# sipposip/pr-disagg-radar-gan

Hardware: AMD Instinct MI355X
Metric: cWGAN-GP train samples/sec, 24x16x16 tiles, bs=256 (higher is better)
Workload: dtype f32; 1 GPU; ndomain=16, 24h, bs=256 fp32, 1 critic step + 1 gen step (BASELINE configs[1]); batch_per_gpu=256, global_batch=256, n_critic=1, parallelism=dp1, world=1, rccl_ranks_seen=1, weights=random init (RandomNormal 0.02 / glorot_uniform), dropout 0.25 active

## Files before the change

### pr_disagg_radar_gan_amd/csrc/rdgan_api.hip

```cpp
#include <hip/hip_runtime.h>
#include <stdio.h>
#include <string.h>
#include <math.h>
#include <string>
#include <vector>
#include <algorithm>
#include <unordered_set>

#include "../../include/rdgan.h"
#include "rdgan_plan.h"
#include "rdgan_hostplan.h"
#include "rdgan_rng.h"
#include "rdgan_gemm.hip.h"
#include "rdgan_gemm_ws.hip.h"
#include "rdgan_gemm_ws16.hip.h"
#include "rdgan_gemm_f16.hip.h"
#include "rdgan_upconv16.hip.h"
#include "rdgan_upconv16b.hip.h"
#include "rdgan_upconv16t.hip.h"
#include "rdgan_elem.hip.h"
#include "rdgan_data.hip.h"
#include "rdgan_edge.hip.h"
#include "rdgan_d2slab16.hip.h"
#include "rdgan_d2fwd16.hip.h"
// ... 63 lines not shown
  int wgrad_boxes = 1;
  int border_boxes = 1;
  int d2_gate_bits = 1;
  int d2_slab = 1;
  int a16 = 0;
  int g9_direct = 1;
  int fast_fwd = -1;
  int fast_bwd = -1;
  float *GWC[4], *GWD[4], *dWc;
  int collapse = 1;
  int tapgather = 1;
  int ws_ksplit = 1;
  int wave_spec = 1;
  int resident = 1;
  int edge_kernels = 1;
  int sample_offset = 0;
  float* g9b_tmp;
  float* gp_part;
  float* dw6_part;
  int side_on = 1;
  int split3 = 0;
  int dense_slices = 0;
  uint64_t gver_in = 0, cver_in = 0;
  const float* gcache_ptr = nullptr; uint64_t gcache_ver = 0; int gcache_cfg = -1;
  const float* ccache_ptr = nullptr; uint64_t ccache_ver = 0; int ccache_cfg = -1;
  long form_builds[2] = {0, 0};
  int keep_gates = 0;
  void* gate_keep[5] = {nullptr, nullptr, nullptr, nullptr, nullptr};
  int gate_keep_B = 0;
  hipStream_t side = nullptr;
  hipEvent_t ev_fork = nullptr, ev_join = nullptr, ev_cw = nullptr, ev_g[4] = {nullptr, nullptr, nullptr, nullptr};
  int* d_flag;
  int fwd_ahead = -1;
  hipStream_t ahead = nullptr;
  hipEvent_t ev_ahead_fork = nullptr, ev_ahead_done = nullptr;
  float* kpartial_ahead = nullptr;
  int* flag_ahead = nullptr;
  bool ahead_pending = false;
  const float *ahead_gp = nullptr, *ahead_z = nullptr, *ahead_cond = nullptr;
  int ahead_B = 0;
  uint64_t ahead_gver = 0;
  std::unordered_set<const void*> lds_attr_done;
  int prof_launches = 0;
  std::vector<RdLaunchRec> launch_recs;
  size_t launch_used = 0;
  char cur_kernel[48] = {0};
  double flops_acc = 0;
  unsigned prof_mask = 0;
  std::vector<hipEvent_t> ev_start[RDGAN_NUM_TAGS], ev_stop[RDGAN_NUM_TAGS];
  size_t ev_used[RDGAN_NUM_TAGS] = {0};
};

#define RD_CHECK(h, call)                                                        \
  do {                                                                           \
    hipError_t e_ = (call);                                                      \
    if (e_ != hipSuccess) {                                                      \
      char b_[512];                                                              \
      snprintf(b_, sizeof b_, "%s:%d %s -> %s", __FILE__, __LINE__, #call, hipGetErrorString(e_)); \
      if (h) (h)->err = b_;                                                      \
      return (int)e_;                                                            \
    }                                                                            \
  } while (0)
#define RD_TRY(expr)            \
  do {                          \
    int r_ = (expr);            \
    if (r_ != 0) return r_;     \
// ... 418 lines not shown
  const bool ws = h && h->wave_spec && !partial && !shift && !dy16 && (h->wave_spec == 2 || wrows * hp.nphases >= 1024 || T.box);
  const bool direct = !ws && !T.box && !dy16 && !partial && np == 1 && nsplit == 1 && h != nullptr && hp.ph[0].w_off == 0;
  if (direct) { T.direct = 1; T.ldw = hp.N; partial_buf = dW; }
  if (dy16) {
    if (shift || BR != 64 || BN != 64) return bad_arg(h, "wgrad: bf16 output gradient only with the 64x64 tile");
    if (partial) RD_TRY((launch_wgrad_cfg<64, 64, true, false, true>(h, dp, np, B, src, dy, partial_buf, T, nsplit, st)));
    else RD_TRY((launch_wgrad_cfg<64, 64, false, false, true>(h, dp, np, B, src, dy, partial_buf, T, nsplit, st)));
  }
  else if (ws && BR == 256) RD_TRY((launch_wgrad_ws_cfg<256, 64>(h, dp, np, B, src, dy, partial_buf, T, nsplit, st)));
  else if (ws && BR == 128 && BN == 128) RD_TRY((launch_wgrad_ws_cfg<128, 128>(h, dp, np, B, src, dy, partial_buf, T, nsplit, st)));
  else if (ws && BR == 128) RD_TRY((launch_wgrad_ws_cfg<128, 64>(h, dp, np, B, src, dy, partial_buf, T, nsplit, st)));
  else if (ws && BN == 128) RD_TRY((launch_wgrad_ws_cfg<64, 128>(h, dp, np, B, src, dy, partial_buf, T, nsplit, st)));
  else if (ws) RD_TRY((launch_wgrad_ws_cfg<64, 64>(h, dp, np, B, src, dy, partial_buf, T, nsplit, st)));
  else if (partial) RD_TRY((launch_wgrad_cfg<64, 64, true, false>(h, dp, np, B, src, dy, partial_buf, T, nsplit, st)));
  else if (BR == 256) RD_WG(256, 64);
  else if (BR == 128 && BN == 128) RD_WG(128, 128);
  else if (BR == 128) RD_WG(128, 64);
  else if (BN == 128) RD_WG(64, 128);
  else RD_WG(64, 64);
#undef RD_WG
  if (direct) { RD_CHECK(h, hipGetLastError()); return 0; }
  if (T.box) {
    const int nw = 64 - __builtin_clzll(hp.wmask | 1ull);
    const long nout = (long)nw * hp.SC * (hp.N / 4);
    hipLaunchKernelGGL(k_wgrad_reduce_box, dim3((unsigned)((nout + 255) / 256)), dim3(256), 0, st, dp, partial_ws, T, BR, B, nw, dW, hp.N);
    RD_CHECK(h, hipGetLastError());
    return 0;
  }
  long total = (long)T.RT * BR * (hp.N / 4);
  int outs = 256;
  while (outs > 16 && (total + outs - 1) / outs * np < 512 && 256 / outs < nsplit) outs >>= 1;
  hipLaunchKernelGGL(k_wgrad_reduce, dim3((unsigned)((total + outs - 1) / outs), np), dim3(256), 0, st, dp, partial_ws,
                     nsplit, T, BR, dW, hp.N, outs);
  RD_CHECK(h, hipGetLastError());
  return 0;
}

template <int BR, int BN>
static int launch_wgrad16_cfg(rdgan_handle* h, const RdPlan* dp, int nphases, int B, const void* src16, const void* dy16,
                              float* partial, const RdWgradTiling& T, int nsplit, hipStream_t st) {
  constexpr size_t lds_loop = ((BR == 256 && BN == 128) ? 3 : 2) * (size_t)(64 * BR * 2 + 64 * BN * 2);
  constexpr size_t lds_epi = (size_t)BR * BN * sizeof(float);
  constexpr size_t lds = lds_loop > lds_epi ? lds_loop : lds_epi;
  auto kern = k_wgrad_gemm_ws16<BR, BN>;
  RD_KNAME(h, "k_wgrad_gemm_ws16<%d,%d>", BR, BN);
  RD_TRY(ensure_lds(h, (const void*)kern, lds));
  dim3 grid((unsigned)(T.box ? T.nsplit : T.RT * T.NT * nsplit * nphases));
  hipLaunchKernelGGL(kern, grid, dim3(512), lds, st, dp, B, (const unsigned short*)src16, (const unsigned short*)dy16, partial, T);
  RD_CHECK(h, hipGetLastError());
  return 0;
}
static bool wgrad16_ok(const RdPlan& hp, int B) {
  int BR, BN, nsplit;
  if (hp.s_shift || hp.SC % 64 || hp.N % 64) return false;
  wgrad_tiling(hp, B, BR, BN, nsplit);
  return BR >= 128;
}
static bool wgrad16_wide(const rdgan_handle* h) { return !h || h->wgrad_wide; }
static int launch_wgrad16(rdgan_handle* h, const RdPlan& hp, const RdPlan* dp, int B, const void* src16, const void* dy16,
                          float* dW, float* partial_ws, size_t partial_cap, hipStream_t st, int tag) {
  ProfScope ps(h, tag, st);
  LaunchScope ls(h, plan_index(h, hp), RD_KIND_WGRAD, B, plan_flops(hp, B), st);
  if (h) h->flops_acc += plan_flops(hp, B);
  if (!wgrad16_ok(hp, B)) return bad_arg(h, "wgrad16: needs SC % 64 == 0, N % 64 == 0, a 128- or 256-row tile, no folded upsample");
  if (!hp.boxes)
  for (int i = 1; i < hp.nphases; ++i)
// ... 337 lines not shown
  if (!strcmp(name, "upconv_slab_t")) { h->upconv_slab_t = value ? 1 : 0; return 0; }
  if (!strcmp(name, "upconv2_slab")) { h->upconv2_slab = value ? 1 : 0; return 0; }
  if (!strcmp(name, "g9_fused")) { h->g9_fused = value ? 1 : 0; return 0; }
  if (!strcmp(name, "d1_fwd_sample")) { h->d1_fwd_sample = value ? 1 : 0; return 0; }
  if (!strcmp(name, "g9_bwd_mfma")) { h->g9_bwd_mfma = value ? 1 : 0; return 0; }
  if (!strcmp(name, "dense16")) { h->dense16 = value ? 1 : 0; return 0; }
  if (!strcmp(name, "dense_skinny")) { h->dense_skinny = value ? 1 : 0; return 0; }
  if (!strcmp(name, "wgrad_boxes")) { h->wgrad_boxes = value ? 1 : 0; return 0; }
  if (!strcmp(name, "border_boxes")) { h->border_boxes = value < 0 ? 0 : (value > 2 ? 2 : value); return 0; }
  if (!strcmp(name, "d3_wgrad_slab")) { h->d3_wgrad_slab = value ? 1 : 0; return 0; }
  if (!strcmp(name, "d2_wgrad_slab")) { h->d2_wgrad_slab = value ? 1 : 0; return 0; }
  if (!strcmp(name, "upwgrad_slab")) { h->upwgrad_slab = value ? 1 : 0; return 0; }
  if (!strcmp(name, "d1_dgrad_fused")) { h->d1_dgrad_fused = value ? 1 : 0; return 0; }
  if (!strcmp(name, "d1_wgrad16")) { h->d1_wgrad16 = value ? 1 : 0; return 0; }
  if (!strcmp(name, "wgrad_wide")) { h->wgrad_wide = value ? 1 : 0; return 0; }
  if (!strcmp(name, "conv_f16")) {
    if (value < 0 || value > 2) return bad_arg(h, "conv_f16: 0, 1 or 2 (2: regardless of the launch size)");
    h->conv_f16 = value; h->ccache_ver = 0; h->gcache_ver = 0; return 0;
  }
  if (!strcmp(name, "d2_fwd_slab")) { h->d2_fwd_slab = value ? 1 : 0; h->ccache_ver = 0; return 0; }
  if (!strcmp(name, "d2_gate_bits")) { h->d2_gate_bits = value ? 1 : 0; return 0; }
  if (!strcmp(name, "d2_slab")) { h->d2_slab = value ? 1 : 0; h->ccache_ver = 0; return 0; }
  if (!strcmp(name, "dense_wgrad_slices")) { h->dense_slices = value; return 0; }
  if (!strcmp(name, "keep_gates")) {
    h->keep_gates = value ? 1 : 0;
    h->gate_keep_B = 0;
    for (int l = 1; l <= 4 && h->keep_gates; ++l)
      if (!h->gate_keep[l]) RD_CHECK(h, hipMalloc(&h->gate_keep[l], (size_t)h->MB * h->dL[l] * h->dch[l] * sizeof(float)));
    return 0;
  }
  if (!strcmp(name, "split3")) { h->split3 = value ? 1 : 0; return 0; }
  if (!strcmp(name, "side_stream")) { h->side_on = (value && h->side) ? 1 : 0; return 0; }
  if (!strcmp(name, "gen_fwd_ahead")) { h->fwd_ahead = value < 0 ? -1 : (value ? 1 : 0); return 0; }
  if (!strcmp(name, "edge_kernels")) { h->edge_kernels = value < 0 ? 0 : (value > 2 ? 2 : value); return 0; }
  if (!strcmp(name, "sample_offset")) { if (value < 0) return bad_arg(h, "set_option: sample_offset < 0"); h->sample_offset = value; return 0; }
  if (!strcmp(name, "ws_ksplit")) { h->ws_ksplit = value < 0 ? 0 : (value > 8 ? 8 : value); return 0; }
  return bad_arg(h, "set_option: unknown option");
}

extern "C" int rdgan_set_weight_versions(rdgan_handle* h, uint64_t gen_version, uint64_t critic_version) {
  if (!h) return -2;
  h->gver_in = gen_version; h->cver_in = critic_version;
  return 0;
}
extern "C" int rdgan_form_builds(const rdgan_handle* h, long* gen_builds, long* critic_builds) {
  if (!h) return -2;
  if (gen_builds) *gen_builds = h->form_builds[0];
  if (critic_builds) *critic_builds = h->form_builds[1];
  return 0;
}

extern "C" int rdgan_profile(rdgan_handle* h, unsigned tag_mask) {
  if (!h) return -2;
  h->prof_mask = tag_mask;
  for (int t = 0; t < RDGAN_NUM_TAGS; ++t) {
    h->ev_used[t] = 0;
    if ((tag_mask >> t & 1u) && h->ev_start[t].empty()) {
      h->ev_start[t].resize(4096); h->ev_stop[t].resize(4096);
      for (size_t i = 0; i < 4096; ++i) {
        RD_CHECK(h, hipEventCreate(&h->ev_start[t][i]));
        RD_CHECK(h, hipEventCreate(&h->ev_stop[t][i]));
      }
    }
  }
  return 0;
}
// ... 1035 lines not shown
      RD_CHECK(h, hipGetLastError());
    } else if (fast) {
      ProfScope ps(h, RDGAN_TAG_ELEMENTWISE, st);
      const long HW = (long)h->gdim[l][1] * h->gdim[l][2];
      RD_TRY(launch_pn_bwd_pairs(h, l == 3 ? h->gh3 : gups[l + 1], hs[l], rs[l], dys[l], h->fgS, (long)B * h->gdim[l - 1][0] * HW,
                                 HW, h->gch[l], st, a16));
    } else {
      ProfScope ps(h, RDGAN_TAG_ELEMENTWISE, st);
      if (l == 3) RD_TRY(launch_pn_bwd(h, h->gh3, hs[3], rs[3], dys[3], npix3, 64, 0, 0, 0, 0, st, a16));
      else RD_TRY(launch_pn_bwd(h, gups[l + 1], hs[l], rs[l], dys[l], (long)B * h->gpix[l], h->gch[l], col ? 0 : 1,
                                h->gdim[l][0], h->gdim[l][1], h->gdim[l][2], st, a16));
    }
    const long cc = (long)h->gch[l - 1] * h->gch[l];
    if (fast) {
      const int* sd = h->gdim[l - 1];
      const int D = sd[0];
      const long P = (long)sd[1] * sd[2] * h->gch[l - 1];
      RdWeightMap wm;
      fastd_weight_map(wm);
      {
        ProfScope ps(h, RDGAN_TAG_ELEMENTWISE, st);
        if (!gen_block_fast(h, l, fast_fwd_on(h))) {
          const dim3 dg(ew_blocks((long)B * (D + 1) * P / 4));
          if (a16) hipLaunchKernelGGL(k_diff_d<rd_bf16_t>, dg, dim3(256), 0, st, (const rd_bf16_t*)hs[l - 1], (rd_bf16_t*)h->fE[l], B, D, P);
          else
          hipLaunchKernelGGL(k_diff_d<float>, dg, dim3(256), 0, st, (const float*)hs[l - 1],
                             h->fE[l], B, D, P);
          hipLaunchKernelGGL(k_weight_transform, dim3(ew_blocks(48L * cc / 4)), dim3(256), 0, st, gp + h->goff[2 * l], h->fU[l],
                             (int)cc, 48, wm);
        }
      }
      const float* wsrc[3] = {h->fE[l], hs[l - 1], h->fE[l]};
      const float* wdy[3] = {dys[l], h->fgS, dys[l]};
      for (int g = 0; g < 3; ++g) {
        int pl = PL_F1WA + 3 * g + l - 1;
        if (!a16 && h->wgrad_boxes && h->border_boxes && h->wave_spec && wgrad_box_ok(h->plans[PL_F1WAX + 3 * g + l - 1]) &&
            (h->border_boxes >= 2 || plan_flops(h->plans[PL_F1WAX + 3 * g + l - 1], 1) < 0.8 * plan_flops(h->plans[pl], 1)))
          pl = PL_F1WAX + 3 * g + l - 1;
        if (a16) {
          if (!wgrad16_ok(h->plans[pl], B)) return bad_arg(h, "bf16 storage mode: no bf16 weight-gradient tile for this block");
          RD_TRY(launch_wgrad16(h, h->plans[pl], h->d_plans + pl, B, wsrc[g], wdy[g], h->fdU, h->wpartial, h->wpartial_cap, st,
                                RDGAN_TAG_GCONV_WGRAD));
        } else
        RD_TRY(launch_wgrad(h, h->plans[pl], h->d_plans + pl, B, wsrc[g], wdy[g], h->fdU, h->wpartial, h->wpartial_cap, st,
                            RDGAN_TAG_GCONV_WGRAD));
      }
      hipLaunchKernelGGL(k_weight_transform_adj, dim3(ew_blocks(27L * cc / 4)), dim3(256), 0, st, h->fdU, grad + h->goff[2 * l],
                         (int)cc, 48, wm);
      RD_TRY(launch_colsum(h, dys[l], (long)B * h->gpix[l], h->gch[l], grad + h->goff[2 * l + 1], side_fork(h, st), a16));
      const int pbs = PL_F1BS + l - 1, pbe = PL_F1BE + l - 1;
      RdEpi eb = epi_make(RD_EPI_PLAIN);
      eb.out16 = a16;
      if (a16) {
        RdSliceMap map;
        fastd_dgrad_slice_map(map.src);
        {
          ProfScope ps(h, RDGAN_TAG_ELEMENTWISE, st);
          hipLaunchKernelGGL(k_blocks_to_bf16, dim3((unsigned)std::min<long>((cc / 8 + 255) / 256, 64), 48), dim3(256), 0, st,
                             h->fU[l], (unsigned short*)h->bUT, cc, map);
        }
        RD_TRY(launch_conv16(h, h->plans[pbs], h->d_plans + pbs, B, h->fgS, h->bUT, gups[l], eb, st, RDGAN_TAG_GCONV_DGRAD));
        RD_TRY(launch_conv16(h, h->plans[pbe], h->d_plans + pbe, B, dys[l], h->bUT, h->fdE, eb, st, RDGAN_TAG_GCONV_DGRAD));
      } else {
        {
          RdSliceMap map;
          fastd_dgrad_slice_map(map.src);
          hipLaunchKernelGGL(k_transpose_map, dim3((h->gch[l] + 31) / 32, (h->gch[l - 1] + 31) / 32, 48), dim3(256), 0, st, h->fU[l],
                             h->fUT, h->gch[l - 1], h->gch[l], map);
        }
        RD_TRY(launch_conv(h, h->plans[pbs], h->d_plans + pbs, B, h->fgS, h->fUT, h->gch[l - 1], gups[l], eb, st,
                           RDGAN_TAG_GCONV_DGRAD));
// ... 983 lines not shown
```

### pr_disagg_radar_gan_amd/csrc/rdgan_gemm.hip.h

```cpp
#pragma once
#include <hip/hip_runtime.h>
#include "rdgan_plan.h"
#include "rdgan_rng.h"
#include <type_traits>

typedef float f32x4 __attribute__((ext_vector_type(4)));
typedef float f32x16 __attribute__((ext_vector_type(16)));
typedef unsigned int u32x4_t __attribute__((ext_vector_type(4)));
typedef unsigned int u32x2_t __attribute__((ext_vector_type(2)));

#define RD_LRELU_ALPHA 0.2f
#ifndef RD_PRIO_LOAD
#define RD_PRIO_LOAD 2
#endif
#define RD_OOB 0x80000000u
#define RD_RSRC_BYTES 0x7FFFFFF0u

typedef unsigned short rd_bf16_t;
typedef __bf16 rd_bf16x2 __attribute__((ext_vector_type(2)));
typedef unsigned int rd_u32x2 __attribute__((ext_vector_type(2)));
__device__ __forceinline__ unsigned rd_pack_bf16(float a, float b) {
  rd_bf16x2 r; r[0] = (__bf16)a; r[1] = (__bf16)b;
  return __builtin_bit_cast(unsigned, r);
}
// ... 779 lines not shown
    __builtin_amdgcn_s_setprio(RD_PRIO_LOAD);
    if (q + 1 < nchunks) store_chunk(buf ^ 1);
    __syncthreads();
  }

  const int N = plan->N;
  if (T.direct) {
#pragma unroll
    for (int i = 0; i < TM; ++i)
#pragma unroll
      for (int r = 0; r < 16; ++r) {
        const int row = wm * WTM + i * 32 + (r & 3) + 8 * (r >> 2) + 4 * lhalf;
        int tap, c;
        rd_wgrad_tile_row(T, BR, rt, row, tap, c);
        if (tap < P.ntaps && c < SC) {
          float* o = partial + ((long)P.tap[tap].w * plan->w_rows_per_tap + c) * T.ldw + n0 + wn * WTN + l31;
#pragma unroll
          for (int j = 0; j < TN; ++j) o[j * 32] = acc[i][j][r];
        }
      }
    return;
  }
  float* out = partial + (((long)bz * T.nsplit + by) * T.RT + rt) * BR * N;
#pragma unroll
  for (int i = 0; i < TM; ++i)
#pragma unroll
    for (int r = 0; r < 16; ++r) {
      const int row = wm * WTM + i * 32 + (r & 3) + 8 * (r >> 2) + 4 * lhalf;
#pragma unroll
      for (int j = 0; j < TN; ++j) out[(long)row * N + n0 + wn * WTN + j * 32 + l31] = acc[i][j][r];
    }
}

__global__ void __launch_bounds__(256)
k_wgrad_reduce(const RdPlan* __restrict__ plan, const float* __restrict__ partial, int nsplit,
               RdWgradTiling T, int BR, float* __restrict__ dW, int ldw, int outs) {
  __shared__ f32x4 red[256];
  const int N = plan->N;
  const int n4s = N / 4;
  const long total = (long)T.RT * BR * n4s;
  const RdPhase& P = plan->ph[blockIdx.y];
  const long stride = (long)T.RT * BR * N;
  const float* pbase = partial + (long)blockIdx.y * nsplit * stride;
  const int ks = 256 / outs, o = threadIdx.x % outs, sl = threadIdx.x / outs;
  const long f = (long)blockIdx.x * outs + o;
  int tap = 0, c = 0, n = 0;
  bool ok = f < total;
  f32x4 s = {0.f, 0.f, 0.f, 0.f};
  if (ok) {
    int R = (int)(f / n4s);
    n = (int)(f - (long)R * n4s) * 4;
    int rt = R / BR, r = R - rt * BR;
    rd_wgrad_tile_row(T, BR, rt, r, tap, c);
    ok = tap < P.ntaps && c < plan->SC;
    if (ok) {
      const float* p = pbase + (long)R * N + n;
      for (int k = sl; k < nsplit; k += ks) s += *(const f32x4*)(p + k * stride);
    }
  }
  if (ks > 1) {
    red[threadIdx.x] = s;
    __syncthreads();
    if (sl == 0)
      for (int j = 1; j < ks; ++j) s += red[j * outs + o];
  }
  if (ok && sl == 0) *(f32x4*)(dW + P.w_off + ((long)P.tap[tap].w * plan->w_rows_per_tap + c) * ldw + n) = s;
}

__global__ void __launch_bounds__(256)
k_wgrad_reduce_box(const RdPlan* __restrict__ plan, const float* __restrict__ partial, RdWgradTiling T, int BR, int B, int nw,
                   float* __restrict__ dW, int ldw) {
  const int N = plan->N, n4s = N / 4, SC = plan->SC;
  const long f = (long)blockIdx.x * 256 + threadIdx.x;
  if (f >= (long)nw * SC * n4s) return;
  const int n = (int)(f % n4s) * 4;
  const int c = (int)((f / n4s) % SC), w = (int)(f / ((long)n4s * SC));
  if (!((plan->wmask >> w) & 1ull)) return;
  f32x4 s0 = {0.f, 0.f, 0.f, 0.f}, s1 = s0;
  int prefix = 0;
  const int np = plan->nphases;
  for (int p = 0; p < np; ++p) {
    const int rtp = rd_wgrad_phase_rt(T, plan->phT[p]);
    const int nsp = (B * plan->phL[p] + (1 << T.rps_log2) - 1) >> T.rps_log2;
    const int k = plan->tapinv[p][w];
    if (k >= 0) {
      int rt, r;
      if (T.tiles_per_tap > 0) { const int ct = c / BR; rt = k * T.tiles_per_tap + ct; r = c - ct * BR; }
      else { rt = k >> T.tpt_log2; r = (k & (T.taps_per_tile - 1)) * T.cw + c; }
      const float* q = partial + ((long)(prefix + rt) * BR + r) * N + n;
      const long st = (long)rtp * BR * N;
      int by = 0;
      for (; by + 1 < nsp; by += 2) { s0 += *(const f32x4*)(q + by * st); s1 += *(const f32x4*)(q + (by + 1) * st); }
      if (by < nsp) s0 += *(const f32x4*)(q + by * st);
    }
    prefix += rtp * nsp;
  }
  *(f32x4*)(dW + plan->ph[0].w_off + ((long)w * plan->w_rows_per_tap + c) * ldw + n) = s0 + s1;
}
```

### pr_disagg_radar_gan_amd/csrc/rdgan_gemm_ws.hip.h

```cpp
#pragma once
#include "rdgan_gemm.hip.h"

#ifndef RD_WGRAD_SCHED
#define RD_WGRAD_SCHED 0
#endif
#ifndef RD_CONV_SCHED
#define RD_CONV_SCHED 0
#endif

#ifdef RD_STAMP
__device__ unsigned long long rd_stamp_ws[8];
#endif
__device__ __forceinline__ void rd_lds_dma16(__amdgpu_buffer_rsrc_t rsrc, float* lds, int voff, int soff) {
  __builtin_amdgcn_raw_ptr_buffer_load_lds(rsrc, (__attribute__((address_space(3))) void*)lds, 16, voff, soff, 0, 0);
}

__device__ __forceinline__ void rd_dma_landed() { asm volatile("s_waitcnt vmcnt(0)" ::: "memory"); }

typedef __bf16 rd_bf16x8 __attribute__((ext_vector_type(8)));
typedef float rd_f32x2 __attribute__((ext_vector_type(2)));
typedef __bf16 rd_bf16x2v __attribute__((ext_vector_type(2)));
__device__ __forceinline__ void rd_split3(const float* x, u32x4_t& p1, u32x4_t& p2, u32x4_t& p3) {
#pragma unroll
  for (int i = 0; i < 4; ++i) {
// ... 533 lines not shown
    const uint32_t ibase = (uint32_t)dbase + epi.idx_base + (uint32_t)(n0 + c4);
#pragma unroll 4
    for (int row = tid / F4R; row < BM; row += RPP) {
      const unsigned rb = Rb[row];
      f32x4 v = *(const f32x4*)&Cs[row * BN + c4];
      if (has_t) v += rd_buf_load4(rsT, Tb[row] + colb);
      if (mode == RD_EPI_BIAS) {
        v += bias4;
      } else if (mode == RD_EPI_BIAS_LRELU || mode == RD_EPI_BIAS_LRELU_DROP) {
        v += bias4;
#pragma unroll
        for (int e = 0; e < 4; ++e) {
          float x = rd_lrelu(v[e]);
          if (mode == RD_EPI_BIAS_LRELU_DROP && epi.use_drop) x = rd_drop_apply_w(x, rd_drop_word(epi.key, ibase + (rb >> 2)), e);
          v[e] = x;
        }
      } else if (mode == RD_EPI_GATE_AUX) {
        const f32x4 a4 = rd_buf_load4(rsX, rb + colb);
#pragma unroll
        for (int e = 0; e < 4; ++e) {
          const float g = rd_gate_from_out(a4[e], epi.use_drop);
          v[e] *= g;
        }
      }
      rd_buf_store4(rsD, rb + colb, v);
    }
  }
#ifdef RD_STAMP
  if (ws_st && wave == 0) atomicAdd(&rd_stamp_ws[3], rd_stamp() - ws_t0);
#endif
}

template <int BR, int BN>
__global__ void __launch_bounds__(512, 4)
k_wgrad_gemm_ws(const RdPlan* __restrict__ plan, int B, const float* __restrict__ src,
                const float* __restrict__ dy, float* __restrict__ partial, RdWgradTiling T) {
  constexpr int BKP = 32;
  constexpr int WTM = BR / 2, WTN = BN / 2, TM = WTM / 32, TN = WTN / 32;
  constexpr int STAGE = BKP * BR + BKP * BN;
  constexpr int A_F4 = BR / 4;
  constexpr int A_PPI = A_F4 >= 64 ? 1 : 64 / A_F4;
  constexpr int A_IPP = A_F4 >= 64 ? A_F4 / 64 : 1;
  static_assert(A_IPP == 1, "BR <= 256");
  constexpr int NI_A = BKP / A_PPI / 4;
  constexpr int B_F4 = BN / 4;
  constexpr int B_PPI = 64 / B_F4;
  constexpr int NI_B = BKP / B_PPI / 4;
  constexpr bool UNI = A_PPI == 1;
  extern __shared__ __attribute__((aligned(16))) float smem[];

  const int tid = threadIdx.x, lane = tid & 63;
  const int wave = __builtin_amdgcn_readfirstlane(tid >> 6);
  const bool is_compute = wave < 4;
  const int l31 = lane & 31, lhalf = lane >> 5;
#ifndef RD_WGRAD_NOPRIO
  __builtin_amdgcn_s_setprio(3);
#endif
  const int swz = rd_xcd_swizzle(blockIdx.x, gridDim.x);
  int by, bz, rt, ntile, slab;
  if (T.box) {
    rd_wgrad_box_decode(plan, T, B, swz, bz, by, rt, ntile, slab);
  } else {
    const int tiles = T.RT * T.NT;
    const int bx = swz % tiles;
    by = (swz / tiles) % T.nsplit; bz = swz / (tiles * T.nsplit);
    rt = bx / T.NT; ntile = bx - rt * T.NT;
    slab = (bz * T.nsplit + by) * T.RT;
  }
  const RdPhase& P = plan->ph[bz];
  const int L = P.L;
  const int rows = B * L;
  const int n0 = ntile * BN;
  const int mbeg = by * T.rows_per_split;
  const int mend = min(rows, mbeg + T.rows_per_split);
  const int nchunks = (mend - mbeg + BKP - 1) / BKP;
  const int N = plan->N;

  f32x16 acc[TM][TN];

  if (!is_compute) {
    const int wl = wave - 4;
    const int SC = plan->SC;
    const int ssample = (int)plan->src_sample, dsample = (int)plan->dst_sample;
    const RdRowTab tab = rd_row_tab(plan, P.tab);
    const int bb0 = mbeg / L;
    const __amdgpu_buffer_rsrc_t rsA = rd_make_rsrc(src + (long)bb0 * plan->src_sample);
    const __amdgpu_buffer_rsrc_t rsB = rd_make_rsrc(dy + (long)bb0 * plan->dst_sample);
    int a_tap, a_c;
    rd_wgrad_tile_row(T, BR, rt, (lane % A_F4) * 4, a_tap, a_c);
    const bool a_ok = a_tap < P.ntaps && a_c < SC;
    int tmask = 0x7FFF, a_const = 0;
// ... 115 lines not shown
            __builtin_amdgcn_sched_group_barrier(0x008, PER, 0);
            __builtin_amdgcn_sched_group_barrier(0x100, 1, 0);
          }
          __builtin_amdgcn_sched_group_barrier(0x008, NMF - PER * NDS > 0 ? NMF - PER * NDS : 0, 0);
        }
#endif
      }
      __syncthreads();
    }
#ifndef RD_WGRAD_NOPRIO
    __builtin_amdgcn_s_setprio(3);
#endif
  }

  float* Cs = smem;
  if (is_compute) {
    const int wm = wave >> 1, wn = wave & 1;
#pragma unroll
    for (int i = 0; i < TM; ++i)
#pragma unroll
      for (int r = 0; r < 16; ++r) {
        const int row = wm * WTM + i * 32 + (r & 3) + 8 * (r >> 2) + 4 * lhalf;
#pragma unroll
        for (int j = 0; j < TN; ++j) Cs[row * BN + wn * WTN + j * 32 + l31] = acc[i][j][r];
      }
  }
  __syncthreads();
  float* out = partial + ((long)slab + rt) * BR * N;
  constexpr int F4R = BN / 4, RPP = 512 / F4R;
  const int c4 = (tid % F4R) * 4;
  for (int row = tid / F4R; row < BR; row += RPP)
    *(f32x4*)(out + (long)row * N + n0 + c4) = *(const f32x4*)&Cs[row * BN + c4];
}
```

### pr_disagg_radar_gan_amd/csrc/rdgan_hostplan.h

```cpp
#pragma once
#include <stdint.h>
#include <stdlib.h>
#include <string.h>
#include <algorithm>
#include <vector>

#include "rdgan_plan.h"

#ifndef RDGAN_NHOURS
#define RDGAN_NHOURS 24
#endif
#ifndef RDGAN_LATENT_DIM
#define RDGAN_LATENT_DIM 100
#endif

static int ilog2(int x) { int l = 0; while ((1 << l) < x) ++l; return l; }

static void phase_defaults(RdPhase& ph, int LD, int LH, int LW) {
  memset(&ph, 0, sizeof(ph));
  ph.LD = LD; ph.LH = LH; ph.LW = LW; ph.L = LD * LH * LW;
  for (int a = 0; a < 3; ++a) { ph.s_mul[a] = 1; ph.o_mul[a] = 1; ph.o_off[a] = 0; }
}

static RdPlan plan_conv_fwd(int D, int H, int W, int Cin, int Cout, int Do, int Ho, int Wo, int stride,
// ... 579 lines not shown
  }
  {
    const int* g3 = h->gdim[3];
    plans[PL_G9F] = plan_rows(g3[0], g3[1], g3[2], 64, 64, 32, 32);
    plans[PL_G9B] = plan_rows(g3[0], g3[1], g3[2], 27, 32, 64, 64);
  }
  plans[PL_D1F] = plan_d1_fwd(nd, h->ddim[1][0], h->ddim[1][1], h->ddim[1][2], h->CP);
  for (int l = 2; l <= 4; ++l) {
    const int* id = h->ddim[l - 1]; const int* od = h->ddim[l]; const int* pd = h->dpad[l - 1];
    plans[PL_D2F + l - 2] = plan_conv_fwd(id[0], id[1], id[2], dch[l - 1], dch[l], od[0], od[1], od[2], 2, pd[0], pd[1], pd[2], 0);
    plans[PL_D2B + l - 2] = plan_conv_dgrad_s2(id[0], id[1], id[2], dch[l - 1], od[0], od[1], od[2], dch[l], pd);
    plans[PL_D2FX + l - 2] = plan_conv_fwd_boxes(id[0], id[1], id[2], dch[l - 1], dch[l], od[0], od[1], od[2], 2, pd[0], pd[1], pd[2]);
    plans[PL_D2BX + l - 2] = plan_boxes(plans[PL_D2B + l - 2]);
  }
  plans[PL_D1B] = plan_rows(h->ddim[1][0], h->ddim[1][1], h->ddim[1][2], 64, 64, h->ldp1, h->ldp1);
  tab.clear();
  first.assign(PL_COUNT, 0);
  for (int i = 0; i < PL_COUNT; ++i) {
    first[i] = tab.size();
    if (!plan_build_tables(plans[i], tab)) return false;
  }
  return true;
}

static const int RD_WGRAD_GEN_PLANS[] = {PL_GDENSE, PL_G1F, PL_G2F, PL_G3F, PL_G9B, PL_G1FC, PL_G2FC, PL_G3FC, PL_G1FCX, PL_G2FCX, PL_G3FCX,
                                         PL_F1WA, PL_F2WA, PL_F3WA, PL_F1WS, PL_F2WS, PL_F3WS, PL_F1WD, PL_F2WD, PL_F3WD,
                                         PL_F1WAX, PL_F2WAX, PL_F3WAX, PL_F1WSX, PL_F2WSX, PL_F3WSX, PL_F1WDX, PL_F2WDX, PL_F3WDX};
static const int RD_WGRAD_CRITIC_PLANS[] = {PL_D1F, PL_D2F, PL_D3F, PL_D4F, PL_D2FX, PL_D3FX, PL_D4FX};

static size_t rd_wgrad_workspace_floats(const RdGeom* h, const std::vector<RdPlan>& plans) {
  size_t wneed = 0;
  for (int id : RD_WGRAD_GEN_PLANS) wneed = std::max(wneed, wgrad_partial_bound(plans[id], h->MB));
  for (int id : RD_WGRAD_CRITIC_PLANS) wneed = std::max(wneed, wgrad_partial_bound(plans[id], h->NB));
  return wneed;
}
```

### pr_disagg_radar_gan_amd/csrc/rdgan_plan.h

```cpp
#pragma once
#include <stdint.h>

#if defined(__HIPCC__)
#define RD_PLAN_HD __host__ __device__ __forceinline__
#else
#define RD_PLAN_HD inline
#endif

#define RD_MAX_TAPS 64
#define RD_MAX_PHASES 32

struct RdTap { int mask, delta, w, code; };

struct RdPhase {
  int L, LD, LH, LW;
  int s_mul[3];
  int s_off[3];
  int o_mul[3], o_off[3];
  int ntaps;
  int w_off;
  int tab;
  int8_t tap_off[RD_MAX_TAPS][4];
  RdTap tap[RD_MAX_TAPS];
};
// ... 23 lines not shown

enum { RD_EPI_PLAIN = 0, RD_EPI_BIAS = 1, RD_EPI_BIAS_LRELU = 2, RD_EPI_BIAS_LRELU_DROP = 3, RD_EPI_GATE_AUX = 4,
       RD_EPI_BIAS_PN_LRELU = 5, RD_EPI_TAPGATHER = 6 };

struct RdEpi {
  int mode;
  int use_drop;
  uint32_t key;
  uint32_t idx_base;
  const float* bias;
  const float* aux;
  int ksplit;
  float* kpart;
  long kstride;
  float* rinv;
  int gw, ghw, gq;
  int nametag;
  const float* addt;
  int addt_plane;
  int out16;
};

struct RdWgradTiling {
  int RT, NT;
  int tiles_per_tap;
  int cw;
  int taps_per_tile;
  int rows_per_split;
  int nsplit, nphases;
  int box, rps_log2, tpt_log2;
  int direct, ldw;
};

RD_PLAN_HD int rd_wgrad_phase_rt(const RdWgradTiling& T, int ntaps) {
  return T.tiles_per_tap > 0 ? ntaps * T.tiles_per_tap : (ntaps + T.taps_per_tile - 1) >> T.tpt_log2;
}

RD_PLAN_HD long rd_wfrag_index(int n, int k, int K) {
  return ((long)(n >> 5) * (K >> 4) + (k >> 4)) * 512 + ((((k >> 3) & 1) << 5) + (n & 31)) * 8 + (k & 7);
}

struct RdWeightMap { int8_t c[48][27]; };
```

Measured before the change: 23810 samples/s.

## Batch three per-layer weight-gradient GEMMs into one grouped launch plus one reduce

The three weight-gradient GEMMs of each generator block (the A/S/D variants), which were launched one after another with a reduce kernel each, now run as one grouped kernel. Each workgroup finds its group from a prefix of first_wg values, and a single 3D reduce kernel folds all three partial buffers. This is meant to cut launch overhead and fill the GPU better, since the small individual grids left compute units idle. In exchange it enlarges the partial workspace to hold three buffers at once, and it falls back to the old path when tilings differ.

```diff
diff --git a/pr_disagg_radar_gan_amd/csrc/rdgan_api.hip b/pr_disagg_radar_gan_amd/csrc/rdgan_api.hip
--- a/pr_disagg_radar_gan_amd/csrc/rdgan_api.hip
+++ b/pr_disagg_radar_gan_amd/csrc/rdgan_api.hip
@@ -119,6 +119,7 @@
   hipEvent_t ev_fork = nullptr, ev_join = nullptr, ev_cw = nullptr, ev_g[4] = {nullptr, nullptr, nullptr, nullptr};
   int* d_flag;
   int fwd_ahead = -1;
+  int wgrad_group = -1;
   hipStream_t ahead = nullptr;
   hipEvent_t ev_ahead_fork = nullptr, ev_ahead_done = nullptr;
   float* kpartial_ahead = nullptr;
@@ -603,6 +604,85 @@
   while (outs > 16 && (total + outs - 1) / outs * np < 512 && 256 / outs < nsplit) outs >>= 1;
   hipLaunchKernelGGL(k_wgrad_reduce, dim3((unsigned)((total + outs - 1) / outs), np), dim3(256), 0, st, dp, partial_ws,
                      nsplit, T, BR, dW, hp.N, outs);
+  RD_CHECK(h, hipGetLastError());
+  return 0;
+}
+
+template <int BR, int BN>
+static int launch_wgrad_ws3_cfg(rdgan_handle* h, const RdWgradGroups& G, unsigned grid, int B, hipStream_t st) {
+  constexpr size_t lds_loop = 2 * (size_t)(32 * BR + 32 * BN) * sizeof(float);
+  constexpr size_t lds_epi = (size_t)BR * BN * sizeof(float);
+  constexpr size_t lds = lds_loop > lds_epi ? lds_loop : lds_epi;
+  auto kern = k_wgrad_gemm_ws3<BR, BN>;
+  RD_KNAME(h, "k_wgrad_gemm_ws3<%d,%d>", BR, BN);
+  RD_TRY(ensure_lds(h, (const void*)kern, lds));
+  hipLaunchKernelGGL(kern, dim3(grid), dim3(512), lds, st, G, B);
+  RD_CHECK(h, hipGetLastError());
+  return 0;
+}
+static bool wgrad_group_on(const rdgan_handle* h) { return h->wgrad_group < 0 ? !h->a16 : h->wgrad_group != 0; }
+
+static int launch_wgrad_group(rdgan_handle* h, const int pl[3], int B, const float* const src[3], const float* const dy[3],
+                              float* dW, hipStream_t st, int tag, bool* taken) {
+  *taken = false;
+  if (!h || !h->wave_spec) return 0;
+  RdWgradGroups G;
+  memset(&G, 0, sizeof(G));
+  int BR0 = 0, BN0 = 0, maxnp = 1;
+  size_t off = 0;
+  unsigned grid = 0;
+  double flops = 0;
+  for (int g = 0; g < 3; ++g) {
+    const RdPlan& hp = h->plans[pl[g]];
+    if (hp.N % 64 || (hp.SC & 3) || hp.s_shift) return 0;
+    if (!hp.boxes)
+      for (int i = 1; i < hp.nphases; ++i)
+        if (hp.ph[i].ntaps != hp.ph[0].ntaps || hp.ph[i].L != hp.ph[0].L) return 0;
+    int BR, BN, nsplit;
+    RdWgradGroup& q = G.g[g];
+    q.T = wgrad_tiling(hp, B, BR, BN, nsplit);
+    if (g == 0) { BR0 = BR; BN0 = BN; }
+    if (BR != BR0 || BN != BN0 || q.T.box != G.g[0].T.box || hp.N != h->plans[pl[0]].N) return 0;
+    if (!(h->wave_spec == 2 || (long)B * hp.ph[0].L * hp.nphases >= 1024 || q.T.box)) return 0;
+    long minL = hp.ph[0].L;
+    for (int i = 1; i < hp.nphases; ++i) minL = std::min<long>(minL, hp.ph[i].L);
+    if (std::min<long>(B, q.T.rows_per_split / minL + 2) * std::max(hp.src_sample, hp.dst_sample) * 4 >= 0x7FFFFFF0L) return 0;
+    const size_t need = q.T.box ? (size_t)q.T.RT * BR * hp.N : (size_t)hp.nphases * nsplit * q.T.RT * BR * hp.N;
+    q.plan = h->d_plans + pl[g]; q.src = src[g]; q.dy = dy[g];
+    q.partial = h->wpartial + off;
+    off += need;
+    q.first_wg = grid;
+    q.nwg = (unsigned)(q.T.box ? q.T.nsplit : q.T.RT * q.T.NT * nsplit * hp.nphases);
+    grid += q.nwg;
+    q.nsplit = nsplit;
+    if (q.T.box) {
+      q.nw = 64 - __builtin_clzll(hp.wmask | 1ull);
+      q.fold_blocks = (int)(((long)q.nw * hp.SC * (hp.N / 4) + 255) / 256);
+    } else {
+      const long total = (long)q.T.RT * BR * (hp.N / 4);
+      int outs = 256;
+      while (outs > 16 && (total + outs - 1) / outs * hp.nphases < 512 && 256 / outs < nsplit) outs >>= 1;
+      q.outs = outs;
+      q.fold_blocks = (int)((total + outs - 1) / outs);
+    }
+    maxnp = std::max(maxnp, hp.nphases);
+    flops += plan_flops(hp, B);
+  }
+  if (off > h->wpartial_cap) return 0;
+  *taken = true;
+  ProfScope ps(h, tag, st);
+  LaunchScope ls(h, pl[0], RD_KIND_WGRAD, B, flops, st);
+  h->flops_acc += flops;
+  if (BR0 == 256) RD_TRY((launch_wgrad_ws3_cfg<256, 64>(h, G, grid, B, st)));
+  else if (BR0 == 128 && BN0 == 128) RD_TRY((launch_wgrad_ws3_cfg<128, 128>(h, G, grid, B, st)));
+  else if (BR0 == 128) RD_TRY((launch_wgrad_ws3_cfg<128, 64>(h, G, grid, B, st)));
+  else if (BN0 == 128) RD_TRY((launch_wgrad_ws3_cfg<64, 128>(h, G, grid, B, st)));
+  else RD_TRY((launch_wgrad_ws3_cfg<64, 64>(h, G, grid, B, st)));
+  const int N = h->plans[pl[0]].N;
+  unsigned fb = 1;
+  for (int g = 0; g < 3; ++g) fb = std::max(fb, (unsigned)G.g[g].fold_blocks);
+  if (G.g[0].T.box) hipLaunchKernelGGL(k_wgrad_reduce_box3, dim3(fb, 1, 3), dim3(256), 0, st, G, BR0, B, dW, N);
+  else hipLaunchKernelGGL(k_wgrad_reduce3, dim3(fb, (unsigned)maxnp, 3), dim3(256), 0, st, G, BR0, dW, N);
   RD_CHECK(h, hipGetLastError());
   return 0;
 }
@@ -1006,6 +1086,7 @@
   if (!strcmp(name, "split3")) { h->split3 = value ? 1 : 0; return 0; }
   if (!strcmp(name, "side_stream")) { h->side_on = (value && h->side) ? 1 : 0; return 0; }
   if (!strcmp(name, "gen_fwd_ahead")) { h->fwd_ahead = value < 0 ? -1 : (value ? 1 : 0); return 0; }
+  if (!strcmp(name, "wgrad_group")) { h->wgrad_group = value < 0 ? -1 : (value ? 1 : 0); return 0; }
   if (!strcmp(name, "edge_kernels")) { h->edge_kernels = value < 0 ? 0 : (value > 2 ? 2 : value); return 0; }
   if (!strcmp(name, "sample_offset")) { if (value < 0) return bad_arg(h, "set_option: sample_offset < 0"); h->sample_offset = value; return 0; }
   if (!strcmp(name, "ws_ksplit")) { h->ws_ksplit = value < 0 ? 0 : (value > 8 ? 8 : value); return 0; }
@@ -2107,11 +2188,18 @@
       }
       const float* wsrc[3] = {h->fE[l], hs[l - 1], h->fE[l]};
       const float* wdy[3] = {dys[l], h->fgS, dys[l]};
+      int wpl[3];
       for (int g = 0; g < 3; ++g) {
         int pl = PL_F1WA + 3 * g + l - 1;
         if (!a16 && h->wgrad_boxes && h->border_boxes && h->wave_spec && wgrad_box_ok(h->plans[PL_F1WAX + 3 * g + l - 1]) &&
             (h->border_boxes >= 2 || plan_flops(h->plans[PL_F1WAX + 3 * g + l - 1], 1) < 0.8 * plan_flops(h->plans[pl], 1)))
           pl = PL_F1WAX + 3 * g + l - 1;
+        wpl[g] = pl;
+      }
+      bool grouped = false;
+      if (!a16 && wgrad_group_on(h)) RD_TRY(launch_wgrad_group(h, wpl, B, wsrc, wdy, h->fdU, st, RDGAN_TAG_GCONV_WGRAD, &grouped));
+      for (int g = 0; g < 3 && !grouped; ++g) {
+        const int pl = wpl[g];
         if (a16) {
           if (!wgrad16_ok(h->plans[pl], B)) return bad_arg(h, "bf16 storage mode: no bf16 weight-gradient tile for this block");
           RD_TRY(launch_wgrad16(h, h->plans[pl], h->d_plans + pl, B, wsrc[g], wdy[g], h->fdU, h->wpartial, h->wpartial_cap, st,
diff --git a/pr_disagg_radar_gan_amd/csrc/rdgan_gemm.hip.h b/pr_disagg_radar_gan_amd/csrc/rdgan_gemm.hip.h
--- a/pr_disagg_radar_gan_amd/csrc/rdgan_gemm.hip.h
+++ b/pr_disagg_radar_gan_amd/csrc/rdgan_gemm.hip.h
@@ -835,18 +835,17 @@
     }
 }
 
-__global__ void __launch_bounds__(256)
-k_wgrad_reduce(const RdPlan* __restrict__ plan, const float* __restrict__ partial, int nsplit,
-               RdWgradTiling T, int BR, float* __restrict__ dW, int ldw, int outs) {
-  __shared__ f32x4 red[256];
+__device__ __forceinline__ void
+rd_wgrad_reduce_body(const RdPlan* __restrict__ plan, const float* __restrict__ partial, int nsplit,
+                     const RdWgradTiling& T, int BR, float* __restrict__ dW, int ldw, int outs, int bx, int phase, f32x4* red) {
   const int N = plan->N;
   const int n4s = N / 4;
   const long total = (long)T.RT * BR * n4s;
-  const RdPhase& P = plan->ph[blockIdx.y];
+  const RdPhase& P = plan->ph[phase];
   const long stride = (long)T.RT * BR * N;
-  const float* pbase = partial + (long)blockIdx.y * nsplit * stride;
+  const float* pbase = partial + (long)phase * nsplit * stride;
   const int ks = 256 / outs, o = threadIdx.x % outs, sl = threadIdx.x / outs;
-  const long f = (long)blockIdx.x * outs + o;
+  const long f = (long)bx * outs + o;
   int tap = 0, c = 0, n = 0;
   bool ok = f < total;
   f32x4 s = {0.f, 0.f, 0.f, 0.f};
@@ -869,12 +868,25 @@
   }
   if (ok && sl == 0) *(f32x4*)(dW + P.w_off + ((long)P.tap[tap].w * plan->w_rows_per_tap + c) * ldw + n) = s;
 }
-
 __global__ void __launch_bounds__(256)
-k_wgrad_reduce_box(const RdPlan* __restrict__ plan, const float* __restrict__ partial, RdWgradTiling T, int BR, int B, int nw,
-                   float* __restrict__ dW, int ldw) {
+k_wgrad_reduce(const RdPlan* __restrict__ plan, const float* __restrict__ partial, int nsplit,
+               RdWgradTiling T, int BR, float* __restrict__ dW, int ldw, int outs) {
+  __shared__ f32x4 red[256];
+  rd_wgrad_reduce_body(plan, partial, nsplit, T, BR, dW, ldw, outs, (int)blockIdx.x, (int)blockIdx.y, red);
+}
+__global__ void __launch_bounds__(256)
+k_wgrad_reduce3(RdWgradGroups G, int BR, float* __restrict__ dW, int ldw) {
+  __shared__ f32x4 red[256];
+  const RdWgradGroup& g = G.g[blockIdx.z];
+  if ((int)blockIdx.x >= g.fold_blocks || (int)blockIdx.y >= g.T.nphases) return;
+  rd_wgrad_reduce_body(g.plan, g.partial, g.nsplit, g.T, BR, dW, ldw, g.outs, (int)blockIdx.x, (int)blockIdx.y, red);
+}
+
+__device__ __forceinline__ void
+rd_wgrad_reduce_box_body(const RdPlan* __restrict__ plan, const float* __restrict__ partial, const RdWgradTiling& T, int BR, int B,
+                         int nw, float* __restrict__ dW, int ldw, int bx) {
   const int N = plan->N, n4s = N / 4, SC = plan->SC;
-  const long f = (long)blockIdx.x * 256 + threadIdx.x;
+  const long f = (long)bx * 256 + threadIdx.x;
   if (f >= (long)nw * SC * n4s) return;
   const int n = (int)(f % n4s) * 4;
   const int c = (int)((f / n4s) % SC), w = (int)(f / ((long)n4s * SC));
@@ -900,3 +912,13 @@
   }
   *(f32x4*)(dW + plan->ph[0].w_off + ((long)w * plan->w_rows_per_tap + c) * ldw + n) = s0 + s1;
 }
+__global__ void __launch_bounds__(256)
+k_wgrad_reduce_box(const RdPlan* __restrict__ plan, const float* __restrict__ partial, RdWgradTiling T, int BR, int B, int nw,
+                   float* __restrict__ dW, int ldw) {
+  rd_wgrad_reduce_box_body(plan, partial, T, BR, B, nw, dW, ldw, (int)blockIdx.x);
+}
+__global__ void __launch_bounds__(256)
+k_wgrad_reduce_box3(RdWgradGroups G, int BR, int B, float* __restrict__ dW, int ldw) {
+  const RdWgradGroup& g = G.g[blockIdx.z];
+  rd_wgrad_reduce_box_body(g.plan, g.partial, g.T, BR, B, g.nw, dW, ldw, (int)blockIdx.x);
+}
diff --git a/pr_disagg_radar_gan_amd/csrc/rdgan_gemm_ws.hip.h b/pr_disagg_radar_gan_amd/csrc/rdgan_gemm_ws.hip.h
--- a/pr_disagg_radar_gan_amd/csrc/rdgan_gemm_ws.hip.h
+++ b/pr_disagg_radar_gan_amd/csrc/rdgan_gemm_ws.hip.h
@@ -589,9 +589,9 @@
 }
 
 template <int BR, int BN>
-__global__ void __launch_bounds__(512, 4)
-k_wgrad_gemm_ws(const RdPlan* __restrict__ plan, int B, const float* __restrict__ src,
-                const float* __restrict__ dy, float* __restrict__ partial, RdWgradTiling T) {
+__device__ __forceinline__ void
+rd_wgrad_gemm_ws_body(const RdPlan* __restrict__ plan, int B, const float* __restrict__ src,
+                      const float* __restrict__ dy, float* __restrict__ partial, const RdWgradTiling& T, int wg, int nwg) {
   constexpr int BKP = 32;
   constexpr int WTM = BR / 2, WTN = BN / 2, TM = WTM / 32, TN = WTN / 32;
   constexpr int STAGE = BKP * BR + BKP * BN;
@@ -613,7 +613,7 @@
 #ifndef RD_WGRAD_NOPRIO
   __builtin_amdgcn_s_setprio(3);
 #endif
-  const int swz = rd_xcd_swizzle(blockIdx.x, gridDim.x);
+  const int swz = rd_xcd_swizzle(wg, nwg);
   int by, bz, rt, ntile, slab;
   if (T.box) {
     rd_wgrad_box_decode(plan, T, B, swz, bz, by, rt, ntile, slab);
@@ -795,3 +795,19 @@
   for (int row = tid / F4R; row < BR; row += RPP)
     *(f32x4*)(out + (long)row * N + n0 + c4) = *(const f32x4*)&Cs[row * BN + c4];
 }
+
+template <int BR, int BN>
+__global__ void __launch_bounds__(512, 4)
+k_wgrad_gemm_ws(const RdPlan* __restrict__ plan, int B, const float* __restrict__ src,
+                const float* __restrict__ dy, float* __restrict__ partial, RdWgradTiling T) {
+  rd_wgrad_gemm_ws_body<BR, BN>(plan, B, src, dy, partial, T, (int)blockIdx.x, (int)gridDim.x);
+}
+
+template <int BR, int BN>
+__global__ void __launch_bounds__(512, 4)
+k_wgrad_gemm_ws3(RdWgradGroups G, int B) {
+  const unsigned wg = blockIdx.x;
+  const int gi = __builtin_amdgcn_readfirstlane((wg >= G.g[1].first_wg ? 1 : 0) + (wg >= G.g[2].first_wg ? 1 : 0));
+  const RdWgradGroup& g = G.g[gi];
+  rd_wgrad_gemm_ws_body<BR, BN>(g.plan, B, g.src, g.dy, g.partial, g.T, (int)(wg - g.first_wg), (int)g.nwg);
+}
diff --git a/pr_disagg_radar_gan_amd/csrc/rdgan_hostplan.h b/pr_disagg_radar_gan_amd/csrc/rdgan_hostplan.h
--- a/pr_disagg_radar_gan_amd/csrc/rdgan_hostplan.h
+++ b/pr_disagg_radar_gan_amd/csrc/rdgan_hostplan.h
@@ -635,5 +635,11 @@
   size_t wneed = 0;
   for (int id : RD_WGRAD_GEN_PLANS) wneed = std::max(wneed, wgrad_partial_bound(plans[id], h->MB));
   for (int id : RD_WGRAD_CRITIC_PLANS) wneed = std::max(wneed, wgrad_partial_bound(plans[id], h->NB));
+  for (int l = 1; l <= 3; ++l) {
+    size_t sum = 0;
+    for (int g = 0; g < 3; ++g)
+      sum += std::max(wgrad_partial_bound(plans[PL_F1WA + 3 * g + l - 1], h->MB), wgrad_partial_bound(plans[PL_F1WAX + 3 * g + l - 1], h->MB));
+    wneed = std::max(wneed, sum);
+  }
   return wneed;
 }
diff --git a/pr_disagg_radar_gan_amd/csrc/rdgan_plan.h b/pr_disagg_radar_gan_amd/csrc/rdgan_plan.h
--- a/pr_disagg_radar_gan_amd/csrc/rdgan_plan.h
+++ b/pr_disagg_radar_gan_amd/csrc/rdgan_plan.h
@@ -79,6 +79,17 @@
   int direct, ldw;
 };
 
+struct RdWgradGroup {
+  const RdPlan* plan;
+  const float* src;
+  const float* dy;
+  float* partial;
+  RdWgradTiling T;
+  unsigned first_wg, nwg;
+  int nsplit, outs, fold_blocks, nw;
+};
+struct RdWgradGroups { RdWgradGroup g[3]; };
+
 RD_PLAN_HD int rd_wgrad_phase_rt(const RdWgradTiling& T, int ntaps) {
   return T.tiles_per_tap > 0 ? ntaps * T.tiles_per_tap : (ntaps + T.taps_per_tile - 1) >> T.tpt_log2;
 }
```

Result: no change. 23990 samples/s, median of 6 (+0.7%).
